# ysbbin/Robust-Object-Detection

Measured on NVIDIA B200. Metric: corrupted images/sec (1360x765 RGB), motion blur k=9, higher is better.
Workload: dtype u8

## Files before the change

robust-object-detection_b200/csrc/blur.cu:

```cuda

#include "rod_internal.h"

namespace rod {

struct BlurParams {
    const DevImage* images;
    const Tile* tiles;
    int n_tiles;
    const uint8_t* src;
    uint8_t* dst;
    const uint8_t* opcodes;
    int k;
    int row_buf_bytes;
    unsigned int* counter;
};

constexpr int kBlurLeft = 64;

__device__ __forceinline__ void cp_async16(uint32_t smem_addr, const void* gptr) {
    asm volatile("cp.async.cg.shared.global [%0], [%1], 16;" ::"r"(smem_addr), "l"(gptr) : "memory");
}
__device__ __forceinline__ void cp_async_wait_all() {
    asm volatile("cp.async.commit_group;\ncp.async.wait_group 0;" ::: "memory");
}
__device__ __forceinline__ void stg16_blur(void* p, uint4 v) {
    asm volatile("st.global.L1::no_allocate.v4.u32 [%0], {%1,%2,%3,%4};" ::"l"(p), "r"(v.x), "r"(v.y), "r"(v.z),
                 "r"(v.w)
                 : "memory");
}

template <int K>
__global__ void __launch_bounds__(256, 4) blur_rows_kernel(BlurParams p) {
    extern __shared__ __align__(16) uint8_t smem[];
    const int warp = threadIdx.x >> 5, lane = threadIdx.x & 31;
    uint8_t* buf = smem + (size_t)warp * p.row_buf_bytes;
    const uint32_t buf_s = (uint32_t)__cvta_generic_to_shared(buf);
    const int k = (K == 0) ? p.k : K;
    const int halo = 3 * (k >> 1);

    for (int sub = 8, ti = 0;;) {
        if (sub >= 8) {
            if (lane == 0) ti = (int)atomicAdd(p.counter, 1u);
            ti = __shfl_sync(0xFFFFFFFFu, ti, 0);
            sub = 0;
        }
        if (ti >= p.n_tiles) break;
        const Tile t = p.tiles[ti];
        const int wr = sub++;
        if (p.opcodes != nullptr && p.opcodes[t.img] != ROD_OP_BLUR) { sub = 8; continue; }
        if (wr >= t.b) { sub = 8; continue; }
        const DevImage im = p.images[t.img];
        const int y = t.a + wr;
        const int n = 3 * im.w;
        const uint8_t* srow = p.src + im.src_off + (int64_t)y * im.src_pitch;
        uint8_t* drow = p.dst + im.dst_off + (int64_t)y * im.dst_pitch;
        const int shift = (int)((uintptr_t)drow & 15);
        uint8_t* row = buf + kBlurLeft + shift;
        const int jf0 = (shift != 0) ? 1 : 0;
        const int jf1 = (n + shift) >> 4;
        const bool right_edge = ((n + shift) & 15) != 0;

        if ((((uintptr_t)srow ^ (uintptr_t)drow) & 15) == 0) {
            const uint8_t* sal = srow - shift;
            for (int j = jf0 + lane; j < jf1; j += 32) cp_async16(buf_s + kBlurLeft + 16 * j, sal + 16 * j);
            const int i = (lane < 16) ? (lane - shift) : (16 * jf1 - shift + lane - 16);
            if (((lane < 16) ? (shift != 0) : right_edge) && i >= 0 && i < n) row[i] = srow[i];
            cp_async_wait_all();
        } else {
            for (int i = lane; i < n; i += 32) row[i] = srow[i];
        }
        __syncwarp();
        if (lane < 2 * halo || K == 0) {
            for (int q = lane; q < 2 * halo; q += 32) {
                const int i = (q < halo) ? (q - halo) : (n + q - halo);
                const int px = (i >= 0) ? i / 3 : -((-i + 2) / 3);
                const int c = i - 3 * px;
                int rp;
                if (im.w > (k >> 1)) rp = (px < 0) ? -px : 2 * (im.w - 1) - px;
                else rp = reflect101(px, im.w);
                row[i] = row[3 * rp + c];
            }
        }
        __syncwarp();
        uint8_t* dal = drow - shift;
        if (K == 9) {
            for (int j = jf0 + lane; j < jf1; j += 32) {
                const uint4* wp = reinterpret_cast<const uint4*>(buf + kBlurLeft + 16 * j - 16);
                const uint4 a = wp[0], b = wp[1], c = wp[2];
                const uint32_t w[12] = {a.x, a.y, a.z, a.w, b.x, b.y, b.z, b.w, c.x, c.y, c.z, c.w};
                uint32_t out[4];
                blur9_chunk16(w, out);
                stg16_blur(dal + 16 * j, make_uint4(out[0], out[1], out[2], out[3]));
            }
            if (lane < 2 && ((lane == 0) ? (shift != 0) : right_edge)) {
                const int j = (lane == 0) ? 0 : jf1;
                const uint4* wp = reinterpret_cast<const uint4*>(buf + kBlurLeft + 16 * j - 16);
                const uint4 a = wp[0], b = wp[1], c = wp[2];
                const uint32_t w[12] = {a.x, a.y, a.z, a.w, b.x, b.y, b.z, b.w, c.x, c.y, c.z, c.w};
                uint32_t out[4];
                blur9_chunk16(w, out);
                const int lo = 16 * j - shift;
                for (int bb = 0; bb < 16; ++bb) {
                    const int i = lo + bb;
                    if (i >= 0 && i < n) drow[i] = (uint8_t)(out[bb >> 2] >> (8 * (bb & 3)));
                }
            }
        } else {
            const int nchunks = (shift + n + 15) >> 4;
            for (int j = lane; j < nchunks; j += 32) {
                const int lo = 16 * j - shift;
                uint32_t out[4];
#pragma unroll
                for (int g = 0; g < 4; ++g) {
                    uint32_t o = 0;
#pragma unroll
                    for (int b = 0; b < 4; ++b) {
                        const int i = lo + 4 * g + b;
                        const uint32_t v = (i >= 0 && i < n) ? blur_byte_generic(row, i, k) : 0u;
                        o |= v << (8 * b);
                    }
                    out[g] = o;
                }
                if (lo >= 0 && lo + 16 <= n) {
                    stg16_blur(dal + 16 * j, make_uint4(out[0], out[1], out[2], out[3]));
                } else {
                    for (int b = 0; b < 16; ++b) {
                        const int i = lo + b;
                        if (i >= 0 && i < n) drow[i] = (uint8_t)(out[b >> 2] >> (8 * (b & 3)));
                    }
                }
            }
        }
        __syncwarp();
    }
}

int launch_blur(const rod_plan* plan, const uint8_t* src, uint8_t* dst, int k, const uint8_t* opcodes,
                cudaStream_t stream, int img_lo, int img_hi) {
    const auto [tiles, n_tiles] = plan->blur_tiles.range(img_lo, img_hi);
    if (n_tiles == 0) return ROD_OK;
    BlurParams p;
    p.images = plan->d_images;
    p.tiles = tiles;
    p.n_tiles = n_tiles;
    p.src = src; p.dst = dst; p.opcodes = opcodes; p.k = k;
    const int row_bytes = 3 * plan->max_w;
    p.row_buf_bytes = kBlurLeft + ((15 + row_bytes + 15) & ~15) + 64;
    int warps = kBlurRowsPerTile;
    while (warps > 1 && (size_t)p.row_buf_bytes * warps > 227 * 1024) --warps;
    const size_t smem = (size_t)p.row_buf_bytes * warps;
    if (smem > 227 * 1024) return ROD_ERR_UNSUPPORTED;
    int ctas_per_sm = (int)((227 * 1024) / (smem + 1024));
    if (ctas_per_sm < 1) ctas_per_sm = 1;
    if (ctas_per_sm > 4) ctas_per_sm = 4;
    p.counter = plan->d_counters + (plan->launch_seq.fetch_add(1u) & (kCounterRing - 1u));
    ROD_CUDA(cudaMemsetAsync(p.counter, 0, sizeof(unsigned int), stream));
    const int grid = grid_for(plan, (p.n_tiles + warps - 1) / warps, ctas_per_sm);
    if (k == 9) {
        ROD_CUDA(cudaFuncSetAttribute(blur_rows_kernel<9>, cudaFuncAttributeMaxDynamicSharedMemorySize, (int)smem));
        blur_rows_kernel<9><<<grid, 32 * warps, smem, stream>>>(p);
    } else {
        ROD_CUDA(cudaFuncSetAttribute(blur_rows_kernel<0>, cudaFuncAttributeMaxDynamicSharedMemorySize, (int)smem));
        blur_rows_kernel<0><<<grid, 32 * warps, smem, stream>>>(p);
    }
    ROD_CUDA(cudaGetLastError());
    return ROD_OK;
}

}
```

robust-object-detection_b200/csrc/plan.cu:

```cuda
#include <map>
#include <new>

#include "rod_internal.h"
#include "rod_tables.h"

namespace rod {

thread_local int g_last_cuda_error = 0;

int grid_for(const rod_plan* plan, int n_tiles, int ctas_per_sm) {
    long long cap = (long long)plan->sm_count * ctas_per_sm;
    return (int)(n_tiles < cap ? n_tiles : cap);
}

static cudaError_t plan_alloc(const rod_plan* plan, void** p, size_t n) {
    const cudaError_t e = block_cache_alloc(plan->device, p, n);
    if (e == cudaSuccess) {
        std::lock_guard<std::mutex> lock(plan->cached_mutex);
        plan->cached_blocks.push_back({*p, n});
    }
    return e;
}
static void plan_free(const rod_plan* plan, void* p) {
    if (p == nullptr) return;
// ... 129 lines not shown
    plan_free(plan, plan->d_tab);
    plan->d_shapes = nullptr;
    plan->d_tab = nullptr;
    int rc = upload(plan, shapes, &plan->d_shapes);
    if (rc == ROD_OK) rc = upload(plan, blob, &plan->d_tab);
    for (int l = 0; l < LR_NUM_LISTS && rc == ROD_OK; ++l) rc = upload_tiles(plan, lists[l], &plan->lowres[l]);
    if (rc != ROD_OK) return rc;
    plan->lowres_x2_smem = x2_smem;
    plan->lowres_factor = factor;
    plan->lowres_all_identity = all_identity;
    plan->lowres_all_x2w = true;
    for (const DevShape& sh : shapes)
        if (!sh.lin_identity && !sh.x2w) plan->lowres_all_x2w = false;
    for (int i = 0; i < plan->n_images; ++i)
        if ((plan->h_images[i].src_pitch & 3) != 0 || (plan->h_images[i].src_off & 3) != 0) plan->lowres_all_x2w = false;
    plan->lowres_half_rows = max_rows;
    plan->lowres_half_cols = max_cols;
    plan->lowres_src_rows = max_src_rows;
    return ROD_OK;
}

int ensure_letterbox_tables(rod_plan* plan, int out_h, int out_w) {
    if (plan->d_lb != nullptr && plan->lb_out_h == out_h && plan->lb_out_w == out_w) return ROD_OK;
    if (out_h < 1 || out_w < 1) return ROD_ERR_INVALID_ARG;
    std::vector<uint32_t> blob;
    std::vector<DevLetterbox> lbs(plan->shapes.size());
    for (size_t s = 0; s < plan->shapes.size(); ++s) {
        DevLetterbox g;
        memset(&g, 0, sizeof(g));
        g.h = plan->shapes[s].h; g.w = plan->shapes[s].w;
        letterbox_geometry(g.h, g.w, out_h, out_w, &g.new_h, &g.new_w, &g.top, &g.left);
        if (g.new_h < 1 || g.new_w < 1 || g.h > 65535 || g.w > 65535) return ROD_ERR_UNSUPPORTED;
        g.identity = (g.new_h == g.h && g.new_w == g.w);
        g.area2 = (!g.identity && g.h == 2 * g.new_h && g.w == 2 * g.new_w);
        if (!g.identity && !g.area2) {
            LinearAxis lx = build_linear_axis(g.w, g.new_w, true);
            LinearAxis ly = build_linear_axis(g.h, g.new_h, false);
            std::vector<uint32_t> ys(g.new_h);
            for (int y = 0; y < g.new_h; ++y) ys[y] = (uint32_t)ly.s0[y] | ((uint32_t)ly.s1[y] << 16);
            g.lx_s0 = blob_push(blob, lx.s0);
            g.lx_a = blob_push(blob, lx.coef);
            g.ly_s = blob_push(blob, ys);
            g.ly_b = blob_push(blob, ly.coef);
            std::vector<uint32_t> pack((size_t)2 * out_w);
            for (int X = 0; X < out_w; ++X) {
                const int cx = X - g.left;
                const bool in = cx >= 0 && cx < g.new_w;
                pack[2 * X] = in ? (uint32_t)(3 * lx.s0[cx]) : 0xFFFFFFFFu;
                pack[2 * X + 1] = in ? lx.coef[cx] : 0u;
            }
            g.lx_pack = blob_push(blob, pack);
            const double stride_words = 2.0 * 3.0 * ((double)g.w / (double)g.new_w) / 4.0;
            g.lane_group = 0;
            for (int pp = 2; pp <= 16; ++pp) {
                const double x = pp * stride_words / 32.0;
                if (fabs(x - nearbyint(x)) * 32.0 < 1.0) { g.lane_group = pp; break; }
            }
        }
        lbs[s] = g;
    }
    if (blob.empty()) blob.push_back(0);
    std::vector<Tile> tiles;
    for (int i = 0; i < plan->n_images; ++i)
        for (int y = 0; y < out_h; y += kLbTH)
            for (int x = 0; x < out_w; x += kLbTW) tiles.push_back(Tile{i, y, x, 0});
    if (plan->d_lb) { plan_free(plan, plan->d_lb); plan->d_lb = nullptr; }
    if (plan->d_lb_tab) { plan_free(plan, plan->d_lb_tab); plan->d_lb_tab = nullptr; }
    int rc = upload(plan, lbs, &plan->d_lb);
    if (rc != ROD_OK) return rc;
    rc = upload(plan, blob, &plan->d_lb_tab);
    if (rc != ROD_OK) return rc;
    rc = upload_tiles(plan, tiles, &plan->lb_tiles);
    if (rc != ROD_OK) return rc;
    plan->lb_all_linear = true;
    for (const DevLetterbox& g : lbs)
        if (g.identity || g.area2) plan->lb_all_linear = false;
    plan->lb_out_h = out_h;
    plan->lb_out_w = out_w;
    return ROD_OK;
}

int ensure_chw_tables(rod_plan* plan) {
    if (plan->d_chw_off != nullptr) return ROD_OK;
    std::vector<Tile> tiles;
    for (int i = 0; i < plan->n_images; ++i)
        for (int y = 0; y < plan->h_images[i].h; y += kChwBandRows)
            tiles.push_back(Tile{i, y, std::min(plan->h_images[i].h, y + kChwBandRows), 0});
    int rc = upload_tiles(plan, tiles, &plan->chw_tiles);
    uint64_t* off = nullptr;
    if (rc == ROD_OK) rc = upload(plan, plan->chw_off, &off);
    if (rc != ROD_OK) {
        plan_free(plan, off);
        return rc;
    }
    plan->d_chw_off = off;
    return ROD_OK;
}

}

using namespace rod;

extern "C" int rod_plan_create(const rod_image_desc* images, int n_images, rod_plan** out_plan) {
    if (out_plan == nullptr) return ROD_ERR_INVALID_ARG;
    *out_plan = nullptr;
    if (images == nullptr || n_images < 1) return ROD_ERR_INVALID_ARG;
    int ndev = 0;
    if (cudaGetDeviceCount(&ndev) != cudaSuccess || ndev == 0) {
        cudaGetLastError();
        return ROD_ERR_NO_DEVICE;
    }
    rod_plan* plan = new (std::nothrow) rod_plan();
    if (plan == nullptr) return ROD_ERR_OOM;
    cudaError_t e = cudaGetDevice(&plan->device);
    if (e == cudaSuccess) e = cudaDeviceGetAttribute(&plan->sm_count, cudaDevAttrMultiProcessorCount, plan->device);
    if (e != cudaSuccess) { delete plan; return cuda_fail(e); }
    plan->n_images = n_images;
    plan->descs.assign(images, images + n_images);
    plan->h_images.resize(n_images);
    std::map<std::pair<int, int>, int> shape_ids;
    uint64_t elem = 0;
    for (int i = 0; i < n_images; ++i) {
        const rod_image_desc& d = images[i];
        if (d.height < 1 || d.width < 1 || d.width > 65535 || d.height > 65535 || d.src_pitch < 3LL * d.width ||
            d.dst_pitch < 3LL * d.width || (uint64_t)d.height * d.width * 3 > 0x7FFFFFFFull) {
            delete plan;
            return ROD_ERR_INVALID_ARG;
        }
        DevImage& im = plan->h_images[i];
        im.src_off = d.src_offset; im.dst_off = d.dst_offset;
        im.src_pitch = d.src_pitch; im.dst_pitch = d.dst_pitch;
        im.h = d.height; im.w = d.width;
        im.elem_base = elem;
        im.contiguous = (d.src_pitch == 3LL * d.width && d.dst_pitch == 3LL * d.width) ? 1 : 0;
        elem += (uint64_t)d.height * d.width * 3;
        auto key = std::make_pair(d.height, d.width);
        auto it = shape_ids.find(key);
        if (it == shape_ids.end()) {
            it = shape_ids.emplace(key, (int)plan->shapes.size()).first;
            plan->shapes.push_back(HostShape{d.height, d.width});
        }
        im.shape_id = it->second;
        plan->max_w = std::max(plan->max_w, d.width);
        plan->all_contiguous = plan->all_contiguous && im.contiguous;
        plan->src_min_offset = (i == 0) ? d.src_offset : std::min<uint64_t>(plan->src_min_offset, d.src_offset);
        plan->src_extent = std::max<uint64_t>(plan->src_extent, d.src_offset + (uint64_t)(d.height - 1) * d.src_pitch + 3ull * d.width);
        plan->dst_extent = std::max<uint64_t>(plan->dst_extent, d.dst_offset + (uint64_t)(d.height - 1) * d.dst_pitch + 3ull * d.width);
    }
    plan->payload_bytes = elem;
    plan->chw_off.resize(n_images + 1);
    plan->chw_off[0] = 0;
    for (int i = 0; i < n_images; ++i)
        plan->chw_off[i + 1] = plan->chw_off[i] + (3ull * images[i].height * images[i].width + 63) / 64 * 64;
    std::vector<Tile> nt, bt;
    build_noise_tiles(plan->h_images, kNoiseSpan, nt);
    build_blur_tiles(plan->h_images, kBlurRowsPerTile, bt);
    for (int i = 1; i < n_images; ++i) {
        const rod_image_desc& a = images[i - 1];
        const rod_image_desc& b = images[i];
        if (b.src_offset < a.src_offset + (uint64_t)a.height * a.src_pitch - (a.src_pitch - 3ull * a.width) ||
            b.dst_offset < a.dst_offset + (uint64_t)a.height * a.dst_pitch - (a.dst_pitch - 3ull * a.width))
            plan->monotonic = false;
    }
    if (plan_alloc(plan, (void**)&plan->d_counters, kCounterRing * sizeof(unsigned int)) != cudaSuccess) { rod_plan_destroy(plan); return ROD_ERR_OOM; }
    int rc = upload(plan, plan->h_images, &plan->d_images);
    if (rc == ROD_OK) rc = upload_tiles(plan, nt, &plan->noise_tiles);
    if (rc == ROD_OK) rc = upload_tiles(plan, bt, &plan->blur_tiles);
    if (rc != ROD_OK) { rod_plan_destroy(plan); return rc; }
    *out_plan = plan;
    return ROD_OK;
}

extern "C" int rod_set_blur_kernel(rod_plan* plan, const float* kernel, int k) {
    if (plan == nullptr) return ROD_ERR_INVALID_ARG;
    if (kernel == nullptr) {
        plan->f2d_ntaps = 0;
        plan->f2d_k = 0;
        return ROD_OK;
    }
    if (k < 1 || (k & 1) == 0) return ROD_ERR_INVALID_ARG;
    if (k * k >= kF2dMaxElems) return ROD_ERR_UNSUPPORTED;
    std::vector<float4> taps;
    for (int dy = 0; dy < k; ++dy)
        for (int dx = 0; dx < k; ++dx) {
            const float w = kernel[dy * k + dx];
            if (w == 0.0f) continue;
            float4 t;
            const int dxb = 3 * dx;
            memcpy(&t.x, &dy, 4);
            memcpy(&t.y, &dxb, 4);
            t.z = w;
            t.w = 0.f;
            taps.push_back(t);
        }
    if (taps.empty()) return ROD_ERR_INVALID_ARG;
    if (plan->d_f2d_taps) { plan_free(plan, plan->d_f2d_taps); plan->d_f2d_taps = nullptr; }
    int rc = upload(plan, taps, &plan->d_f2d_taps);
    if (rc != ROD_OK) return rc;
    if (plan->f2d_tiles.d == nullptr) {
        std::vector<Tile> tiles;
        build_grid_tiles(plan->h_images, kF2dTH, kF2dTWB, tiles);
        rc = upload_tiles(plan, tiles, &plan->f2d_tiles);
        if (rc != ROD_OK) return rc;
    }
    plan->f2d_ntaps = (int)taps.size();
    plan->f2d_k = k;
    return ROD_OK;
}

extern "C" void rod_plan_destroy(rod_plan* plan) {
    if (plan == nullptr) return;
    if (plan->inner) rod_plan_destroy(plan->inner);
    cudaDeviceSynchronize();
    if (plan->d_patch_clean) cudaFree(plan->d_patch_clean);
    if (plan->d_patch_corrupted) cudaFree(plan->d_patch_corrupted);
    void* ptrs[] = {plan->d_images, plan->noise_tiles.d, plan->blur_tiles.d, plan->d_shapes, plan->d_tab, plan->d_lb,
                    plan->d_lb_tab, plan->lb_tiles.d, plan->d_scratch, plan->d_stage_src, plan->d_f2d_taps,
                    plan->f2d_tiles.d, plan->d_counters, plan->d_stage_dst, plan->d_stage_noise, plan->d_stage_ops,
                    plan->chw_tiles.d, plan->d_chw_off};
    for (void* p : ptrs) plan_free(plan, p);
    for (const TileList& l : plan->lowres) plan_free(plan, l.d);
    for (cudaStream_t s : plan->streams)
        if (s) cudaStreamDestroy(s);
    for (cudaStream_t s : plan->aux_streams)
        if (s) cudaStreamDestroy(s);
    for (cudaStream_t s : plan->lr_streams)
        if (s) cudaStreamDestroy(s);
    if (plan->lr_ev_fork) cudaEventDestroy(plan->lr_ev_fork);
    for (cudaEvent_t e : plan->lr_ev_join)
        if (e) cudaEventDestroy(e);
    if (plan->ev_fork) cudaEventDestroy(plan->ev_fork);
    for (cudaEvent_t e : plan->ev_join)
        if (e) cudaEventDestroy(e);
    delete plan;
}

extern "C" int rod_plan_num_images(const rod_plan* plan) { return plan ? plan->n_images : 0; }
extern "C" uint64_t rod_plan_payload_bytes(const rod_plan* plan) { return plan ? plan->payload_bytes : 0; }
extern "C" uint64_t rod_plan_chw_offset(const rod_plan* plan, int i) {
    return (plan != nullptr && i >= 0 && i <= plan->n_images) ? plan->chw_off[i] : 0;
}
```

robust-object-detection_b200/csrc/rod_core.h:

```cpp
#pragma once
#include <math.h>
#include <stdint.h>
#include <string.h>

#if defined(__CUDACC__)
#define ROD_HD __host__ __device__ __forceinline__
#else
#define ROD_HD inline
#endif

namespace rod {

struct DevImage {
    uint64_t src_off, dst_off;
    int64_t src_pitch, dst_pitch;
    uint64_t elem_base;
    int32_t h, w;
    int32_t shape_id;
    int32_t contiguous;
};

struct Tile {
    int32_t img, a, b, c;
};

enum AreaMode { AREA_GENERAL = 0, AREA_FAST2 = 1, AREA_FASTN = 2, AREA_IDENTITY = 3 };

struct DevShape {
    int32_t h, w, nh, nw;
    int32_t area_mode;
    int32_t ix, iy;
    int32_t xt, yt;
    uint32_t ax_first, ax_alpha;
    uint32_t ay_first, ay_alpha;
    uint32_t ax_count, ay_count;
    uint32_t lx_s0, lx_a;
    uint32_t ly_s, ly_b;
    float inv_area;
    int32_t lin_identity;
    int32_t x2;
    int32_t strip_rows;
    int32_t strip_half_rows;
    uint32_t ay_pack;
    int32_t ay_packed;
    uint32_t ly_rc;
    int32_t x2w;
    int32_t x2p;
    uint32_t ly_rc2;
    uint32_t ly_rc3;
    int32_t x2g;
    uint32_t hy_pack;
    int32_t x2h;
    int32_t x2i;
};

#if defined(__CUDA_ARCH__)
ROD_HD float fmul(float a, float b) { return __fmul_rn(a, b); }
ROD_HD float fadd(float a, float b) { return __fadd_rn(a, b); }
ROD_HD float frint(float a) { return rintf(a); }
ROD_HD float fadd_rz(float a, float b) { return __fadd_rz(a, b); }
ROD_HD uint32_t fbits(float a) { return __float_as_uint(a); }
ROD_HD float bitsf(uint32_t a) { return __uint_as_float(a); }
#else
ROD_HD float fmul(float a, float b) { volatile float r = a * b; return r; }
ROD_HD float fadd(float a, float b) { volatile float r = a + b; return r; }
ROD_HD float frint(float a) { return nearbyintf(a); }
ROD_HD float fadd_rz(float a, float b) { return (float)floor((double)a + (double)b); }
ROD_HD uint32_t fbits(float a) { uint32_t u; memcpy(&u, &a, 4); return u; }
ROD_HD float bitsf(uint32_t a) { float f; memcpy(&f, &a, 4); return f; }
#endif

ROD_HD int reflect101(int i, int n) {
    if (n == 1) return 0;
    int period = 2 * (n - 1);
    int m = i % period;
    if (m < 0) m += period;
    return m < n ? m : period - m;
}

ROD_HD uint32_t noise_px(float vf, float nz) {
    float s = fadd(vf, nz);
    s = fmaxf(s, 0.0f);
    s = fminf(s, 255.0f);
    return fbits(fadd_rz(s, 8388608.0f)) & 0xFFu;
}

ROD_HD uint32_t mulhi32(uint32_t a, uint32_t b) {
#if defined(__CUDA_ARCH__)
    return __umulhi(a, b);
#else
    return (uint32_t)(((uint64_t)a * (uint64_t)b) >> 32);
#endif
}

ROD_HD void philox4x32_10(uint32_t c0, uint32_t c1, uint32_t c2, uint32_t c3, uint32_t k0, uint32_t k1,
                          uint32_t r[4]) {
#pragma unroll
    for (int i = 0; i < 10; ++i) {
        uint32_t hi0 = mulhi32(0xD2511F53u, c0), lo0 = 0xD2511F53u * c0;
        uint32_t hi1 = mulhi32(0xCD9E8D57u, c2), lo1 = 0xCD9E8D57u * c2;
        uint32_t n0 = hi1 ^ c1 ^ k0;
        uint32_t n2 = hi0 ^ c3 ^ k1;
        c0 = n0; c1 = lo1; c2 = n2; c3 = lo0;
        k0 += 0x9E3779B9u; k1 += 0xBB67AE85u;
    }
    r[0] = c0; r[1] = c1; r[2] = c2; r[3] = c3;
}

struct PhiloxKeys {
    uint32_t rk[20];
};
inline PhiloxKeys philox_round_keys(uint32_t k0, uint32_t k1) {
    PhiloxKeys ks;
    for (int i = 0; i < 10; ++i) {
        ks.rk[2 * i] = k0 + (uint32_t)i * 0x9E3779B9u;
        ks.rk[2 * i + 1] = k1 + (uint32_t)i * 0xBB67AE85u;
    }
    return ks;
}
template <int ROUNDS>
ROD_HD void philox4x32_rk(uint32_t c0, uint32_t c1, uint32_t c2, uint32_t c3, const PhiloxKeys& ks, uint32_t r[4]) {
#if defined(__CUDA_ARCH__)
#pragma unroll
#endif
    for (int i = 0; i < ROUNDS; ++i) {
        uint32_t hi0 = mulhi32(0xD2511F53u, c0), lo0 = 0xD2511F53u * c0;
        uint32_t hi1 = mulhi32(0xCD9E8D57u, c2), lo1 = 0xCD9E8D57u * c2;
        uint32_t n0 = hi1 ^ c1 ^ ks.rk[2 * i];
        uint32_t n2 = hi0 ^ c3 ^ ks.rk[2 * i + 1];
        c0 = n0; c1 = lo1; c2 = n2; c3 = lo0;
    }
    r[0] = c0; r[1] = c1; r[2] = c2; r[3] = c3;
}
ROD_HD void philox4x32_10_rk(uint32_t c0, uint32_t c1, uint32_t c2, uint32_t c3, const PhiloxKeys& ks, uint32_t r[4]) {
    philox4x32_rk<10>(c0, c1, c2, c3, ks, r);
}

#define ROD_PHILOX_TAIL_FLIP 0x80000000u
#define ROD_NOISE_K_PER_SIGMA 1.17741002251547466f
#define ROD_ANGLE_SCALE 9.58737992428525768e-05f
#define ROD_ANGLE_BIAS (-804.247680664062500f)
ROD_HD bool philox_needs_tail(const uint32_t r[4]) {
    uint32_t m = r[0] < r[1] ? r[0] : r[1];
    const uint32_t m2 = r[2] < r[3] ? r[2] : r[3];
    m = m < m2 ? m : m2;
    return m < 0x10000u;
}
ROD_HD void gauss2(uint32_t rw, bool use_tail, uint32_t tw, float* s0, float* s1) {
#if defined(__CUDA_ARCH__)
    const float xh = bitsf(__byte_perm(rw, 0x4B000000u, 0x7432));
    const float xl = bitsf(__byte_perm(rw, 0x4B000000u, 0x7410));
    float u = fmaf(xh, 1.52587890625e-05f, -127.99999237060546875f);
    if (use_tail && rw < 0x10000u) u = fmaf((float)tw, 3.5527136788005009e-15f, 1.7763568394002505e-15f);
    float l2, rad;
    asm("lg2.approx.ftz.f32 %0, %1;" : "=f"(l2) : "f"(u));
    asm("sqrt.approx.ftz.f32 %0, %1;" : "=f"(rad) : "f"(-l2));
    const float th = fmaf(xl, ROD_ANGLE_SCALE, ROD_ANGLE_BIAS);
    *s0 = rad * __cosf(th);
    *s1 = rad * __sinf(th);
#else
    double u = ((double)(rw >> 16) + 0.5) * 1.52587890625e-05;
    if (use_tail && rw < 0x10000u) u = ((double)tw + 0.5) * 3.5527136788005009e-15;
    const double rad = sqrt(-log2(u));
    const double th = (8388608.0 + (double)(rw & 0xFFFFu)) * (double)ROD_ANGLE_SCALE + (double)ROD_ANGLE_BIAS;
    *s0 = (float)(rad * cos(th));
    *s1 = (float)(rad * sin(th));
#endif
}
ROD_HD void gauss8(const uint32_t r[4], const uint32_t* t, float s[8]) {
#if defined(__CUDA_ARCH__)
#pragma unroll
#endif
    for (int p = 0; p < 4; ++p) gauss2(r[p], t != nullptr, t != nullptr ? t[p] : 0u, &s[2 * p], &s[2 * p + 1]);
}
ROD_HD uint32_t noise_floor16(float s, float K) {
#if defined(__CUDA_ARCH__)
    return fbits(__fmaf_rd(s, K, 12582912.0f));
// ... 520 lines not shown
```

robust-object-detection_b200/csrc/rod_internal.h:

```cpp
#pragma once
#include <cuda_runtime.h>

#include <atomic>
#include <mutex>
#include <utility>
#include <vector>

#include "../../include/rod_b200.h"
#include "rod_core.h"

namespace rod {

constexpr unsigned int kCounterRing = 4096;

constexpr int kNoiseSpan = 16384;
constexpr int kBlurRowsPerTile = 8;
constexpr int kLowresTH = 32;
constexpr int kLowresTWB = 480;
constexpr int kLbTH = 32;
constexpr int kLbTW = 64;
constexpr int kMaxAreaTaps = 8;
constexpr int kF2dTH = 16;
constexpr int kF2dTWB = 768;
constexpr int kF2dMaxElems = 130;
constexpr int kChwBandRows = 8;

struct HostShape {
    int h, w;
};

struct DevLetterbox {
    int32_t h, w, new_h, new_w, top, left;
    int32_t area2;
    int32_t identity;
    uint32_t lx_s0, lx_a;
    uint32_t ly_s, ly_b;
    uint32_t lx_pack;
    int32_t lane_group;
};

struct TileList {
    Tile* d = nullptr;
    int n = 0;
    std::vector<int> start;
    std::pair<const Tile*, int> range(int lo, int hi) const {
        if (n == 0) return {d, 0};
        return {d + start[lo], start[hi] - start[lo]};
    }
};

enum LowresList {
    LR_GENERIC,
    LR_X2_STRIP,
    LR_X2_REST,
    LR_X2W8, LR_X2W4,
    LR_X2P16, LR_X2P8, LR_X2P4,
    LR_X2F16, LR_X2F8, LR_X2F4,
    LR_X2H16, LR_X2H8, LR_X2H4,
    LR_X2G,
    LR_X2I_CARRY, LR_X2I_EVEN,
    LR_NUM_LISTS
};

}

struct rod_plan {
    int device = 0;
    int n_images = 0;
    int sm_count = 148;
    std::vector<rod_image_desc> descs;
    std::vector<rod::DevImage> h_images;
    std::vector<rod::HostShape> shapes;
    uint64_t payload_bytes = 0;
    int max_w = 0;
    bool all_contiguous = true;
    uint64_t src_extent = 0, dst_extent = 0;
    uint64_t src_min_offset = 0;

    rod::DevImage* d_images = nullptr;
    rod::TileList noise_tiles, blur_tiles;
    rod::TileList lowres[rod::LR_NUM_LISTS];
    size_t lowres_x2_smem = 0;
    unsigned int* d_counters = nullptr;
    mutable std::atomic<unsigned int> launch_seq{0};
    bool monotonic = true;
    int gauss_generator = ROD_GAUSS_AUTO;

    double lowres_factor = -1.0;
    rod::DevShape* d_shapes = nullptr;
    uint32_t* d_tab = nullptr;
    bool lowres_all_identity = false;
    bool lowres_all_x2w = false;
    int lowres_half_rows = 0, lowres_half_cols = 0;
    int lowres_src_rows = 0;

    int lb_out_h = 0, lb_out_w = 0;
    rod::DevLetterbox* d_lb = nullptr;
    uint32_t* d_lb_tab = nullptr;
    bool lb_all_linear = false;
    rod::TileList lb_tiles;
    uint8_t* d_scratch = nullptr;
    uint64_t scratch_bytes = 0;

    std::vector<uint64_t> chw_off;
    uint64_t* d_chw_off = nullptr;
    rod::TileList chw_tiles;

    float4* d_f2d_taps = nullptr;
    int f2d_ntaps = 0, f2d_k = 0;
    rod::TileList f2d_tiles;

    rod_plan* inner = nullptr;
    uint8_t* d_patch_clean = nullptr;
    uint8_t* d_patch_corrupted = nullptr;

    uint8_t* d_stage_src = nullptr;
    uint8_t* d_stage_dst = nullptr;
    float* d_stage_noise = nullptr;
    uint8_t* d_stage_ops = nullptr;
    cudaStream_t streams[3] = {nullptr, nullptr, nullptr};
    cudaStream_t aux_streams[2] = {nullptr, nullptr};
    cudaEvent_t ev_fork = nullptr, ev_join[2] = {nullptr, nullptr};
    mutable std::mutex cached_mutex;
    mutable std::vector<std::pair<void*, size_t>> cached_blocks;
    mutable std::mutex lr_mutex;
    mutable cudaStream_t lr_streams[2] = {nullptr, nullptr};
    mutable cudaEvent_t lr_ev_fork = nullptr, lr_ev_join[2] = {nullptr, nullptr};
};

namespace rod {
extern thread_local int g_last_cuda_error;
inline int cuda_fail(cudaError_t e) {
    g_last_cuda_error = (int)e;
    return e == cudaErrorMemoryAllocation ? ROD_ERR_OOM : ROD_ERR_CUDA;
}
#define ROD_CUDA(call)                                  \
    do {                                                \
        cudaError_t _e = (call);                        \
        if (_e != cudaSuccess) return rod::cuda_fail(_e); \
    } while (0)

int grid_for(const rod_plan* plan, int n_tiles, int ctas_per_sm);

cudaError_t block_cache_alloc(int dev, void** p, size_t n);
void block_cache_free(int dev, void* p, size_t n);

int launch_noise(const rod_plan* plan, int mode, const uint8_t* src, uint8_t* dst, const float* noise,
                 float* field_out, float sigma, uint64_t seed, uint64_t first_image, uint32_t offset,
                 const uint8_t* opcodes, int my_op, cudaStream_t stream, int img_lo, int img_hi,
                 int generator = -1 );
int launch_blur(const rod_plan* plan, const uint8_t* src, uint8_t* dst, int k, const uint8_t* opcodes,
                cudaStream_t stream, int img_lo, int img_hi);
int launch_lowres(const rod_plan* plan, const uint8_t* src, uint8_t* dst, const uint8_t* opcodes,
                  cudaStream_t stream, int img_lo, int img_hi);
int launch_filter2d(const rod_plan* plan, const uint8_t* src, uint8_t* dst, const uint8_t* opcodes, cudaStream_t stream,
                    int img_lo, int img_hi);
int launch_gather_patches(const rod_plan* plan, const rod_plan* inner, const uint8_t* src, uint8_t* clean,
                          const uint8_t* flips, cudaStream_t stream);
int launch_resize_linear(const uint8_t* src, int h, int w, int64_t src_pitch, uint8_t* dst, int nh, int nw, int64_t dst_pitch,
                         cudaStream_t stream);
int launch_format_pairs(const rod_plan* inner, const uint8_t* clean, const uint8_t* corrupted, float* clean_out,
                        float* corrupted_out, cudaStream_t stream);
int launch_fused_letterbox(const rod_plan* plan, const uint8_t* src, const uint8_t* scratch, const uint8_t* opcodes,
                           const float* noise, void* out_f16, int pad_value, float sigma, int k, uint64_t seed,
                           uint64_t first_image, uint32_t offset, bool lowres_in_kernel, cudaStream_t stream);
int launch_letterbox(const rod_plan* plan, const uint8_t* img, const uint8_t* src, const uint8_t* opcodes, void* out_f16,
                     int pad_value, cudaStream_t stream);
int launch_chw_f32(const rod_plan* plan, const uint8_t* src, const uint8_t* scratch, const uint8_t* opcodes, float* out,
                   cudaStream_t stream);

int gauss_table_for(int device, float sigma, const int32_t** out);
int ensure_lowres_tables(rod_plan* plan, double factor);
int ensure_letterbox_tables(rod_plan* plan, int out_h, int out_w);
int ensure_chw_tables(rod_plan* plan);

enum NoiseMode { NOISE_COMPAT = 0, NOISE_PHILOX = 1, NOISE_COPY = 2, NOISE_FIELD = 3 };
}
```

robust-object-detection_b200/csrc/rod_tables.h:

```cpp
#pragma once
#include <math.h>
#include <stdint.h>
#include <string.h>

#include <algorithm>
#include <vector>

#include "rod_core.h"

namespace rod {

struct AreaAxis {
    std::vector<int32_t> first, count;
    std::vector<float> alpha;
    int taps = 1;
};

inline AreaAxis build_area_axis(int ssize, int dsize) {
    AreaAxis ax;
    ax.first.assign(dsize, 0);
    ax.count.assign(dsize, 0);
    std::vector<std::vector<float>> rows(dsize);
    double scale = (double)ssize / (double)dsize;
    for (int d = 0; d < dsize; ++d) {
// ... 131 lines not shown
                int na = 0, nb = 0;
                while (r < h && ly.s1[r] == j && ly.s0[r] == j - 1) { ++na; ++r; }
                while (r < h && ly.s1[r] == j && ly.s0[r] == j) { ++nb; ++r; }
                if (na > 255 || nb > 255 || r0 > 65535) return false;
                const uint32_t* pk = blob.data() + sh.ay_pack + 4 * (size_t)j;
                hp[4 * j] = pk[1]; hp[4 * j + 1] = pk[2]; hp[4 * j + 2] = pk[3];
                hp[4 * j + 3] = (uint32_t)r0 | ((uint32_t)na << 16) | ((uint32_t)nb << 24);
            }
            if (r != h) return false;
            sh.hy_pack = blob_push(blob, hp);
            return true;
        };
        if (sh.area_mode == AREA_GENERAL && sh.ay_packed && sh.xt == 3 && w == 2 * sh.nw + 1 && sh.nw >= 1 && h >= 2) {
            const int32_t* xf = (const int32_t*)(blob.data() + sh.ax_first);
            const int32_t* xc = (const int32_t*)(blob.data() + sh.ax_count);
            bool ok = true;
            for (int dx = 0; dx < sh.nw && ok; ++dx) ok = (xf[dx] == 2 * dx && xc[dx] == 3);
            for (int x = 0; x < w && ok; ++x) {
                const int i = (x & 1) ? (x - 1) / 2 : x / 2 - 1;
                ok = (x & 1) ? (lx.s0[x] == i || (i >= 1 && lx.s0[x] == i - 1)) : (lx.s0[x] == std::max(i, 0));
            }
            if (ok) {
                std::vector<float> rc3((size_t)h * 4);
                for (int y = 0; y < h; ++y) {
                    const X2Row r = x2g_row_consts(ly.coef[y]);
                    rc3[4 * y] = r.c0s; rc3[4 * y + 1] = r.c1s; rc3[4 * y + 2] = r.k0; rc3[4 * y + 3] = r.k2;
                }
                sh.ly_rc3 = blob_push(blob, rc3);
                sh.x2g = 1;
                if (build_row_schedule(3)) sh.x2i = 1;
                else if (build_row_schedule(2)) sh.x2i = 2;
            }
        }
        if (sh.x2) {
            std::vector<float> rc((size_t)h * 4);
            for (int y = 0; y < h; ++y) {
                const X2Row r = x2_row_consts(ly.coef[y]);
                rc[4 * y] = r.c0s; rc[4 * y + 1] = r.c1s; rc[4 * y + 2] = r.k0; rc[4 * y + 3] = r.k2;
            }
            sh.ly_rc = blob_push(blob, rc);
            std::vector<uint32_t> rc2((size_t)h * 4);
            for (int y = 0; y < h; ++y) {
                const X2Row r = x2_row_consts(ly.coef[y]);
                const float k0p = r.k0 + 2.0f;
                memcpy(&rc2[4 * y], &r.c0s, 4); memcpy(&rc2[4 * y + 1], &r.c1s, 4); memcpy(&rc2[4 * y + 2], &k0p, 4);
                rc2[4 * y + 3] = x2_vertical_cfix(ly.coef[y]);
            }
            sh.ly_rc2 = blob_push(blob, rc2);
            sh.x2w = ((w & 3) == 0 && h >= 2 && (sh.area_mode == AREA_FAST2 || (sh.area_mode == AREA_GENERAL && sh.ay_packed))) ? 1 : 0;
            bool packed = sh.x2w && sh.area_mode == AREA_FAST2;
            for (int y = 0; y < h && packed; ++y) {
                const int s0 = (y & 1) ? (y - 1) / 2 : std::max(y / 2 - 1, 0);
                const int s1 = (y & 1) ? std::min(s0 + 1, sh.nh - 1) : y / 2;
                const uint32_t coef = (y & 1) ? (1536u | (512u << 16)) : (512u | (1536u << 16));
                packed = (ly.s0[y] == s0 && ly.s1[y] == s1 && ly.coef[y] == coef);
            }
            sh.x2p = packed ? 1 : 0;
            if (sh.x2w && sh.area_mode == AREA_GENERAL && sh.ay_packed && build_row_schedule(3)) sh.x2h = 1;
        }
    }
    *out = sh;
    return true;
}

inline size_t choose_strip_rows(DevShape* sh, const uint32_t* blob) {
    const size_t max_smem = 54 * 1024;
    const int nthreads = 128;
    sh->strip_rows = 0;
    sh->strip_half_rows = 0;
    if (!sh->x2 || sh->lin_identity) return 0;
    const size_t pitch = (size_t)((3 * sh->nw + 24 + 15) & ~15);
    const uint32_t* ly = blob + sh->ly_s;
    const int nchunks = (sh->w + 7) / 8;
    double best = -1.0;
    size_t best_smem = 0;
    for (int R = 16; R <= 64; R += 8) {
        int nj = 1;
        for (int y0 = 0; y0 < sh->h; y0 += R) {
            const int y1 = std::min(sh->h, y0 + R) - 1;
            nj = std::max(nj, (int)(ly[y1] >> 16) - (int)(ly[y0] & 0xFFFF) + 1);
        }
        const size_t smem = (size_t)nj * pitch;
        if (smem > max_smem) continue;
        const int rows = std::min(R, sh->h);
        const int items = ((rows + 7) / 8) * nchunks;
        const double fill = (double)items / (double)(((items + nthreads - 1) / nthreads) * nthreads);
        const double apron = (double)rows / (2.0 * nj);
        const double score = fill * std::min(1.0, apron);
        if (score > best + 1e-9) { best = score; sh->strip_rows = R; sh->strip_half_rows = nj; best_smem = smem; }
    }
    return best_smem;
}

inline void build_strip_tiles(const std::vector<DevImage>& imgs, const std::vector<DevShape>& shapes, bool want_x2,
                              int th, int twb, std::vector<Tile>& tiles) {
    for (int i = 0; i < (int)imgs.size(); ++i) {
        const DevShape& sh = shapes[imgs[i].shape_id];
        const bool is_x2 = sh.strip_rows > 0;
        if (is_x2 != want_x2) continue;
        if (is_x2) {
            for (int y = 0; y < imgs[i].h; y += sh.strip_rows) tiles.push_back(Tile{i, y, 0, 0});
        } else {
            for (int y = 0; y < imgs[i].h; y += th)
                for (int b = 0; b < 3 * imgs[i].w; b += twb) tiles.push_back(Tile{i, y, b, 0});
        }
    }
}

inline void letterbox_geometry(int h, int w, int out_h, int out_w, int* new_h, int* new_w, int* top, int* left) {
    double r = std::min((double)out_h / h, (double)out_w / w);
    *new_w = (int)nearbyint(w * r);
    *new_h = (int)nearbyint(h * r);
    double dw = (out_w - *new_w) / 2.0, dh = (out_h - *new_h) / 2.0;
    *top = (int)nearbyint(dh - 0.1);
    *left = (int)nearbyint(dw - 0.1);
}

inline void build_gauss_table(float sigma, int32_t* X) {
    double y[256], q[257], ph[257];
    for (int i = 128; i <= 256; ++i) {
        q[i] = (i == 256) ? 0.0 : (i == 128 ? 0.0 : -ndtri_double((256 - i) / 256.0));
        ph[i] = (i == 256) ? 0.0 : exp(-0.5 * q[i] * q[i]) * 0.39894228040143267794;
    }
    double m2 = 0.0;
    for (int i = 128; i < 256; ++i) {
        const double z = 256.0 * (ph[i] - ph[i + 1]);
        const double z4 = (z * z) * (z * z);
        y[i] = z * (1.0 + ROD_GAUSS_H4_STRETCH_A * z4 + ROD_GAUSS_H4_STRETCH_B * (z4 * z4));
        m2 += y[i] * y[i];
    }
    const double norm = 128.0 * (double)sigma / sqrt(m2 / 128.0);
    for (int i = 128; i < 256; ++i) {
        X[i] = (int32_t)floor(norm * y[i] + 0.5);
        X[255 - i] = -X[i];
    }
}

inline void build_noise_tiles(const std::vector<DevImage>& imgs, int span, std::vector<Tile>& tiles) {
    for (int i = 0; i < (int)imgs.size(); ++i) {
        const DevImage& im = imgs[i];
        int64_t row = 3LL * im.w;
        if (im.contiguous) {
            int64_t n = row * im.h;
            for (int64_t e = 0; e < n; e += span)
                tiles.push_back(Tile{i, (int32_t)e, (int32_t)std::min<int64_t>(span, n - e), -1});
        } else {
            for (int y = 0; y < im.h; ++y)
                for (int64_t e = 0; e < row; e += span)
                    tiles.push_back(Tile{i, (int32_t)e, (int32_t)std::min<int64_t>(span, row - e), y});
        }
    }
}

inline void build_blur_tiles(const std::vector<DevImage>& imgs, int rows_per_tile, std::vector<Tile>& tiles) {
    for (int i = 0; i < (int)imgs.size(); ++i)
        for (int y = 0; y < imgs[i].h; y += rows_per_tile)
            tiles.push_back(Tile{i, y, std::min(rows_per_tile, imgs[i].h - y), 0});
}

inline void build_grid_tiles(const std::vector<DevImage>& imgs, int th, int twb, std::vector<Tile>& tiles) {
    for (int i = 0; i < (int)imgs.size(); ++i)
        for (int y = 0; y < imgs[i].h; y += th)
            for (int b = 0; b < 3 * imgs[i].w; b += twb) tiles.push_back(Tile{i, y, b, 0});
}

inline void lowres_tile_footprint(const DevShape& sh, const uint32_t* blob, int th, int twb, int* rows, int* cols,
                                  int* src_rows = nullptr) {
    const int32_t* lx = (const int32_t*)(blob + sh.lx_s0);
    const uint32_t* ly = blob + sh.ly_s;
    const int32_t* yf = (const int32_t*)(blob + sh.ay_first);
    const int32_t* yc = (const int32_t*)(blob + sh.ay_count);
    int mr = 1, mc = 1, ms = 1;
    for (int y0 = 0; y0 < sh.h; y0 += th) {
        const int y1 = std::min(sh.h, y0 + th) - 1;
        const int j_lo = (int)(ly[y0] & 0xFFFF), j_hi = (int)(ly[y1] >> 16);
        mr = std::max(mr, j_hi - j_lo + 1);
        if (sh.area_mode == AREA_GENERAL) ms = std::max(ms, yf[j_hi] + yc[j_hi] - yf[j_lo]);
        else ms = std::max(ms, (j_hi - j_lo + 1) * sh.iy);
    }
    for (int b0 = 0; b0 < 3 * sh.w; b0 += twb) {
        const int x0 = b0 / 3, x1 = (std::min(3 * sh.w, b0 + twb) - 1) / 3;
        mc = std::max(mc, std::min(lx[x1] + 1, sh.nw - 1) - lx[x0] + 1);
    }
    *rows = mr;
    *cols = mc;
    if (src_rows) *src_rows = ms;
}

}
```

Measured before the change: 945,000.

## Replace blur tile list with prefix-row claiming and self-resetting counters

Blur work is no longer taken from a precomputed tile array. Warps atomically claim spans of 8 global rows and map each row to its image by binary search over a per-image first-row prefix table. The per-launch cudaMemsetAsync of the work counter is removed: the last warp to finish resets the slot pair itself, which saves one stream operation per launch. In exchange the kernel takes on a completion-count protocol that has to be correct, plus a search step whenever a warp claims a new span.

```diff
diff --git a/robust-object-detection_b200/csrc/blur.cu b/robust-object-detection_b200/csrc/blur.cu
--- a/robust-object-detection_b200/csrc/blur.cu
+++ b/robust-object-detection_b200/csrc/blur.cu
@@ -5,14 +5,15 @@
 
 struct BlurParams {
     const DevImage* images;
-    const Tile* tiles;
-    int n_tiles;
+    const uint32_t* first_row;
+    int img_lo, img_hi;
+    uint32_t row_lo, rows;
     const uint8_t* src;
     uint8_t* dst;
     const uint8_t* opcodes;
     int k;
     int row_buf_bytes;
-    unsigned int* counter;
+    unsigned int* slot;
 };
 
 constexpr int kBlurLeft = 64;
@@ -38,19 +39,38 @@
     const int k = (K == 0) ? p.k : K;
     const int halo = 3 * (k >> 1);
 
-    for (int sub = 8, ti = 0;;) {
-        if (sub >= 8) {
-            if (lane == 0) ti = (int)atomicAdd(p.counter, 1u);
-            ti = __shfl_sync(0xFFFFFFFFu, ti, 0);
-            sub = 0;
+    const uint32_t warps = gridDim.x * (blockDim.x >> 5);
+    uint32_t r = 0, r_end = 0, img_first = 0, img_end = 0;
+    int img = 0;
+    for (;;) {
+        if (r >= r_end) {
+            uint32_t s = 0;
+            if (lane == 0) s = atomicAdd(p.slot, kBlurClaimRows);
+            s = __shfl_sync(0xFFFFFFFFu, s, 0);
+            if (s >= p.rows) {
+                if (lane == 0) {
+                    __threadfence();
+                    if (atomicAdd(p.slot + 1, 1u) == warps - 1u) {
+                        __threadfence();
+                        p.slot[0] = 0u;
+                        p.slot[1] = 0u;
+                    }
+                }
+                break;
+            }
+            r = p.row_lo + s;
+            r_end = p.row_lo + min(p.rows, s + kBlurClaimRows);
+            img = blur_row_image(p.first_row, p.img_lo, p.img_hi, r);
+            img_first = p.first_row[img];
+            img_end = p.first_row[img + 1];
         }
-        if (ti >= p.n_tiles) break;
-        const Tile t = p.tiles[ti];
-        const int wr = sub++;
-        if (p.opcodes != nullptr && p.opcodes[t.img] != ROD_OP_BLUR) { sub = 8; continue; }
-        if (wr >= t.b) { sub = 8; continue; }
-        const DevImage im = p.images[t.img];
-        const int y = t.a + wr;
+        while (r >= img_end) {
+            img_first = img_end;
+            img_end = p.first_row[++img + 1];
+        }
+        if (p.opcodes != nullptr && p.opcodes[img] != ROD_OP_BLUR) { r = min(r_end, img_end); continue; }
+        const DevImage im = p.images[img];
+        const int y = (int)(r++ - img_first);
         const int n = 3 * im.w;
         const uint8_t* srow = p.src + im.src_off + (int64_t)y * im.src_pitch;
         uint8_t* drow = p.dst + im.dst_off + (int64_t)y * im.dst_pitch;
@@ -137,25 +157,27 @@
 
 int launch_blur(const rod_plan* plan, const uint8_t* src, uint8_t* dst, int k, const uint8_t* opcodes,
                 cudaStream_t stream, int img_lo, int img_hi) {
-    const auto [tiles, n_tiles] = plan->blur_tiles.range(img_lo, img_hi);
-    if (n_tiles == 0) return ROD_OK;
+    if (plan->d_first_row == nullptr) return ROD_ERR_UNSUPPORTED;
+    const uint32_t row_lo = (uint32_t)plan->first_row[img_lo];
+    const uint32_t rows = (uint32_t)plan->first_row[img_hi] - row_lo;
+    if (rows == 0) return ROD_OK;
     BlurParams p;
     p.images = plan->d_images;
-    p.tiles = tiles;
-    p.n_tiles = n_tiles;
+    p.first_row = plan->d_first_row;
+    p.img_lo = img_lo; p.img_hi = img_hi;
+    p.row_lo = row_lo; p.rows = rows;
     p.src = src; p.dst = dst; p.opcodes = opcodes; p.k = k;
     const int row_bytes = 3 * plan->max_w;
     p.row_buf_bytes = kBlurLeft + ((15 + row_bytes + 15) & ~15) + 64;
-    int warps = kBlurRowsPerTile;
+    int warps = kBlurWarps;
     while (warps > 1 && (size_t)p.row_buf_bytes * warps > 227 * 1024) --warps;
     const size_t smem = (size_t)p.row_buf_bytes * warps;
     if (smem > 227 * 1024) return ROD_ERR_UNSUPPORTED;
     int ctas_per_sm = (int)((227 * 1024) / (smem + 1024));
     if (ctas_per_sm < 1) ctas_per_sm = 1;
     if (ctas_per_sm > 4) ctas_per_sm = 4;
-    p.counter = plan->d_counters + (plan->launch_seq.fetch_add(1u) & (kCounterRing - 1u));
-    ROD_CUDA(cudaMemsetAsync(p.counter, 0, sizeof(unsigned int), stream));
-    const int grid = grid_for(plan, (p.n_tiles + warps - 1) / warps, ctas_per_sm);
+    p.slot = plan->d_blur_slots + 2 * (plan->blur_seq.fetch_add(1u) & (kCounterRing - 1u));
+    const int grid = grid_for(plan, (int)((rows + 8u * warps - 1u) / (8u * warps)), ctas_per_sm);
     if (k == 9) {
         ROD_CUDA(cudaFuncSetAttribute(blur_rows_kernel<9>, cudaFuncAttributeMaxDynamicSharedMemorySize, (int)smem));
         blur_rows_kernel<9><<<grid, 32 * warps, smem, stream>>>(p);
diff --git a/robust-object-detection_b200/csrc/plan.cu b/robust-object-detection_b200/csrc/plan.cu
--- a/robust-object-detection_b200/csrc/plan.cu
+++ b/robust-object-detection_b200/csrc/plan.cu
@@ -305,9 +305,11 @@
     plan->chw_off[0] = 0;
     for (int i = 0; i < n_images; ++i)
         plan->chw_off[i + 1] = plan->chw_off[i] + (3ull * images[i].height * images[i].width + 63) / 64 * 64;
-    std::vector<Tile> nt, bt;
+    std::vector<Tile> nt;
     build_noise_tiles(plan->h_images, kNoiseSpan, nt);
-    build_blur_tiles(plan->h_images, kBlurRowsPerTile, bt);
+    plan->first_row.resize(n_images + 1);
+    plan->first_row[0] = 0;
+    for (int i = 0; i < n_images; ++i) plan->first_row[i + 1] = plan->first_row[i] + (uint64_t)images[i].height;
     for (int i = 1; i < n_images; ++i) {
         const rod_image_desc& a = images[i - 1];
         const rod_image_desc& b = images[i];
@@ -318,7 +320,9 @@
     if (plan_alloc(plan, (void**)&plan->d_counters, kCounterRing * sizeof(unsigned int)) != cudaSuccess) { rod_plan_destroy(plan); return ROD_ERR_OOM; }
     int rc = upload(plan, plan->h_images, &plan->d_images);
     if (rc == ROD_OK) rc = upload_tiles(plan, nt, &plan->noise_tiles);
-    if (rc == ROD_OK) rc = upload_tiles(plan, bt, &plan->blur_tiles);
+    if (rc == ROD_OK) rc = upload(plan, std::vector<unsigned int>(2 * kCounterRing, 0u), &plan->d_blur_slots);
+    if (rc == ROD_OK && plan->first_row[n_images] <= 0x7FFFFFFFull)
+        rc = upload(plan, std::vector<uint32_t>(plan->first_row.begin(), plan->first_row.end()), &plan->d_first_row);
     if (rc != ROD_OK) { rod_plan_destroy(plan); return rc; }
     *out_plan = plan;
     return ROD_OK;
@@ -367,7 +371,7 @@
     cudaDeviceSynchronize();
     if (plan->d_patch_clean) cudaFree(plan->d_patch_clean);
     if (plan->d_patch_corrupted) cudaFree(plan->d_patch_corrupted);
-    void* ptrs[] = {plan->d_images, plan->noise_tiles.d, plan->blur_tiles.d, plan->d_shapes, plan->d_tab, plan->d_lb,
+    void* ptrs[] = {plan->d_images, plan->noise_tiles.d, plan->d_first_row, plan->d_blur_slots, plan->d_shapes, plan->d_tab, plan->d_lb,
                     plan->d_lb_tab, plan->lb_tiles.d, plan->d_scratch, plan->d_stage_src, plan->d_f2d_taps,
                     plan->f2d_tiles.d, plan->d_counters, plan->d_stage_dst, plan->d_stage_noise, plan->d_stage_ops,
                     plan->chw_tiles.d, plan->d_chw_off};
diff --git a/robust-object-detection_b200/csrc/rod_core.h b/robust-object-detection_b200/csrc/rod_core.h
--- a/robust-object-detection_b200/csrc/rod_core.h
+++ b/robust-object-detection_b200/csrc/rod_core.h
@@ -23,6 +23,17 @@
 struct Tile {
     int32_t img, a, b, c;
 };
+
+constexpr uint32_t kBlurClaimRows = 8;
+
+ROD_HD int blur_row_image(const uint32_t* first_row, int lo, int hi, uint32_t r) {
+    while (hi - lo > 1) {
+        const int m = (lo + hi) >> 1;
+        if (first_row[m] <= r) lo = m;
+        else hi = m;
+    }
+    return lo;
+}
 
 enum AreaMode { AREA_GENERAL = 0, AREA_FAST2 = 1, AREA_FASTN = 2, AREA_IDENTITY = 3 };
 
diff --git a/robust-object-detection_b200/csrc/rod_internal.h b/robust-object-detection_b200/csrc/rod_internal.h
--- a/robust-object-detection_b200/csrc/rod_internal.h
+++ b/robust-object-detection_b200/csrc/rod_internal.h
@@ -14,7 +14,7 @@
 constexpr unsigned int kCounterRing = 4096;
 
 constexpr int kNoiseSpan = 16384;
-constexpr int kBlurRowsPerTile = 8;
+constexpr int kBlurWarps = 8;
 constexpr int kLowresTH = 32;
 constexpr int kLowresTWB = 480;
 constexpr int kLbTH = 32;
@@ -78,11 +78,15 @@
     uint64_t src_min_offset = 0;
 
     rod::DevImage* d_images = nullptr;
-    rod::TileList noise_tiles, blur_tiles;
+    rod::TileList noise_tiles;
+    std::vector<uint64_t> first_row;
+    uint32_t* d_first_row = nullptr;
     rod::TileList lowres[rod::LR_NUM_LISTS];
     size_t lowres_x2_smem = 0;
     unsigned int* d_counters = nullptr;
     mutable std::atomic<unsigned int> launch_seq{0};
+    unsigned int* d_blur_slots = nullptr;
+    mutable std::atomic<unsigned int> blur_seq{0};
     bool monotonic = true;
     int gauss_generator = ROD_GAUSS_AUTO;
 
diff --git a/robust-object-detection_b200/csrc/rod_tables.h b/robust-object-detection_b200/csrc/rod_tables.h
--- a/robust-object-detection_b200/csrc/rod_tables.h
+++ b/robust-object-detection_b200/csrc/rod_tables.h
@@ -307,12 +307,6 @@
     }
 }
 
-inline void build_blur_tiles(const std::vector<DevImage>& imgs, int rows_per_tile, std::vector<Tile>& tiles) {
-    for (int i = 0; i < (int)imgs.size(); ++i)
-        for (int y = 0; y < imgs[i].h; y += rows_per_tile)
-            tiles.push_back(Tile{i, y, std::min(rows_per_tile, imgs[i].h - y), 0});
-}
-
 inline void build_grid_tiles(const std::vector<DevImage>& imgs, int th, int twb, std::vector<Tile>& tiles) {
     for (int i = 0; i < (int)imgs.size(); ++i)
         for (int y = 0; y < imgs[i].h; y += th)
```

Measured after the change: 947,600 (median of 6 runs). Within noise of the previous version (+0.3%).
